# gpuopenanalytics/libgdf

Measured on AMD Instinct MI355X. Metric: hash-join probe rows/s, higher is better.
Workload: dtype int64

## Files before the change

### include/gdf/gdf_amd_testhook.h

```cpp
#ifndef GDF_AMD_TESTHOOK_H
#define GDF_AMD_TESTHOOK_H
#include "gdf/gdf.h"
#ifdef __cplusplus
extern "C" {
#endif
gdf_error gdf_amd_debug_force(const char *name, const char *value);
const char *gdf_amd_testhook_forced(const char *name);
void gdf_amd_testhook_note(const char *name, long long value);
gdf_error gdf_amd_debug_noted(const char *name, long long *value);
#ifdef __cplusplus
}
#endif
#endif
```

### libgdf_amd/csrc/join.hip

```cpp
#include "internal.h"
#include "launch.h"
#include "gdf/gdf_amd_ext.h"

#include <cmath>
#include <cstdio>

#include <algorithm>
#include <cstdlib>
#include <deque>
#include <memory>
#include <type_traits>
#include <vector>

namespace gdf_amd {

enum KeyMode : int { KM_RAW_INT = 0, KM_RAW_FLOAT, KM_PACKED, KM_HASHED };

struct KeyPlan {
  int mode;
  int verify;
  int narrow;
  uint64_t kmin;
  uint64_t kspan;
  uint64_t klimit;
  uint64_t kwindow;
  int shift[MAX_KEY_COLS];
  int ranged;
  int bits[MAX_KEY_COLS];
  long long bias[MAX_KEY_COLS];
};

static KeyPlan plan_keys(const KeyTable &t) {
  KeyPlan p{};
  bool all_int = true;
  int total = 0;
  for (int c = 0; c < t.ncols; ++c) {
    if (t.col[c].kind == K_F32 || t.col[c].kind == K_F64) all_int = false;
    p.shift[c] = total * 8;
    total += t.col[c].width;
  }
  if (t.ncols == 1) p.mode = all_int ? KM_RAW_INT : KM_RAW_FLOAT;
  else if (all_int && total <= 8) p.mode = KM_PACKED;
  else { p.mode = KM_HASHED; p.verify = 1; }
  if (p.mode != KM_HASHED && total <= 4) p.narrow = 1;
  p.klimit = p.narrow ? 0xffffffffULL : ~0ULL;
  return p;
}

__device__ __forceinline__ bool float_bits(const ColView &c, int64_t i, uint64_t &bits) {
  if (c.kind == K_F32) {
    uint32_t b = ((const uint32_t *)c.data)[i];
    if ((b & 0x7fffffffu) > 0x7f800000u) return false;
    if ((b << 1) == 0) b = 0;
    bits = b;
  } else {
    uint64_t b = ((const uint64_t *)c.data)[i];
    if ((b & 0x7fffffffffffffffULL) > 0x7ff0000000000000ULL) return false;
    if ((b << 1) == 0) b = 0;
    bits = b;
  }
  return true;
}

__device__ __forceinline__ long long load_int_signed(const ColView &c, int64_t i) {
  switch (c.width) {
    case 1: return ((const int8_t *)c.data)[i];
    case 2: return ((const int16_t *)c.data)[i];
    case 4: return ((const int32_t *)c.data)[i];
    default: return ((const long long *)c.data)[i];
  }
}

__device__ __forceinline__ bool make_key(const KeyTable &t, const KeyPlan &p, int64_t i, uint64_t &key) {
  if (!row_valid(t, i)) return false;
  switch (p.mode) {
    case KM_RAW_INT: {
      const uint64_t k = load_bits(t.col[0], i) - p.kmin;
      key = k;
      return k <= p.klimit;
    }
    case KM_RAW_FLOAT: return float_bits(t.col[0], i, key);
    case KM_PACKED: {
      uint64_t k = 0;
// ... 815 lines not shown
    uint32_t claimed = 0;
    {
      const uint32_t tid = opaque_tid();
      if (g.cap1 && tid < ncoarse) {
        const uint32_t cnt = s.hist[tid];
        if (cnt) claimed = atomicAdd(&g.spec_cursor1[(tid << g.xs) | (blockIdx.x & ((1u << g.xs) - 1u))], cnt);
      }
      tile_scan_bins(s, ncoarse, tid);
      block_sync();
    }
    const uint32_t wtid = opaque_tid();
    {
      uint32_t st[ITEMS];
#pragma unroll
      for (int k = 0; k < ITEMS; ++k) st[k] = s.start[(binrank[k] >> 16) & 255u];
#pragma unroll
      for (int k = 0; k < ITEMS; ++k) {
        const uint32_t pos = (okmask >> k) & 1u ? st[k] + (binrank[k] & 0xffffu) : (uint32_t)TILE;
        const int32_t row = g.row_base + (int32_t)(tile + item_row(k, wtid));
        s.w[pos] = ((uint64_t)key[k] << 32) | (uint32_t)row;
        if constexpr (PMODE == 4) *reinterpret_cast<ulonglong2 *>(&s.pay[2 * (size_t)pos]) = ulonglong2{pay[k], pay2[k]};
        else s.pay[pos] = pay[k];
      }
    }
    {
      const uint32_t tid = opaque_tid();
      if (tid < ncoarse) {
        if (g.cap1) {
          const uint32_t cnt = s.hist[tid];
          const uint32_t region = (tid << g.xs) | (blockIdx.x & ((1u << g.xs) - 1u));
          if (claimed + cnt > g.cap1) { atomicExch(g.spec_flag, 1u); s.gbase[tid] = g.dump - s.start[tid]; }
          else s.gbase[tid] = region * g.cap1 + claimed - s.start[tid];
        } else {
          s.gbase[tid] = s.cursor[tid] - s.start[tid];
          s.cursor[tid] += s.hist[tid];
        }
      }
      if (tid < 256) s.hist[tid] = 0;
      if (g.cap1 && tid == 0) s.total_abort = __hip_atomic_load(g.spec_flag, __ATOMIC_RELAXED, __HIP_MEMORY_SCOPE_AGENT);
    }
    const bool more = tile + TILE < end;
    __builtin_amdgcn_sched_barrier(0);
    if (more) prefetch(tile + TILE);
    block_sync();
    if (g.cap1 && s.total_abort) return;
    const uint32_t total = s.total;
    const uint32_t ftid = opaque_tid();
    constexpr int GROUP = ITEMS % 4 == 0 ? 4 : 3;
#pragma unroll
    for (int h = 0; h < ITEMS / GROUP; ++h) {
      uint64_t ww[GROUP], pp[GROUP], pq[PMODE == 4 ? GROUP : 1];
      uint32_t gb[GROUP];
#pragma unroll
      for (int k = 0; k < GROUP; ++k) {
        const uint32_t j = ftid + (h * GROUP + k) * THREADS;
        ww[k] = s.w[j];
        if constexpr (PMODE == 4) { const ulonglong2 e = *reinterpret_cast<const ulonglong2 *>(&s.pay[2 * (size_t)j]); pp[k] = e.x; pq[k] = e.y; }
        else pp[k] = s.pay[j];
      }
#pragma unroll
      for (int k = 0; k < GROUP; ++k) gb[k] = s.gbase[(fine_of((ww[k] >> 32) + g.kbias, g.fb) >> g.b2) & 255u];
#pragma unroll
      for (int k = 0; k < GROUP; ++k) {
        const uint32_t j = ftid + (h * GROUP + k) * THREADS;
        const uint32_t dst = j < total ? gb[k] + j : g.dump + ftid;
        out.w[dst] = ww[k];
        if constexpr (PMODE == 4) *reinterpret_cast<ulonglong2 *>(out.pay + 2 * (size_t)dst) = ulonglong2{pp[k], pq[k]};
        else out.pay[dst] = pp[k];
      }
      __builtin_amdgcn_sched_barrier(0);
    }
    consume(tile + TILE);
    __builtin_amdgcn_sched_barrier(0);
  }
}

struct Level2Map {
  const uint32_t *coarse_off;
  const uint32_t *coarse_end;
  const uint32_t *tile_prefix;
  int xs;
  uint32_t ntiles;
  int xcd_order;
  const uint32_t *ntiles_dev;
  uint32_t nseg;
  const uint32_t *keys32;
  uint32_t calib_step;
};
static inline uint32_t sc2_grid(const Level2Map &m, uint32_t ntiles) {
  const uint32_t tiles = m.calib_step > 1 ? (ntiles + m.calib_step - 1) / m.calib_step : ntiles;
  return m.xcd_order ? ((tiles + 7) / 8) * 8 : tiles;
}

template <bool NARROW, int THREADS, int PAY = 0, bool P6 = false, bool K32 = false, bool IN6 = false, int NITEMS = 0>
__global__ __launch_bounds__(THREADS) void jk_scatter2(PartGeom g, Level2Map m, Tuples in,
                                                             uint32_t *__restrict__ fine_cursor, Tuples out) {
  extern __shared__ __attribute__((aligned(16))) unsigned char tile_raw[];
  constexpr int ITEMS = NITEMS ? NITEMS : (PAY ? JK_PAY_ITEMS : JK_SC_ITEMS);
  using Tile = TileLds<NARROW, THREADS, PAY, ITEMS>;
  Tile &s = *reinterpret_cast<Tile *>(tile_raw);
  constexpr int JK_TILE = THREADS * ITEMS;
  const uint32_t ncoarse = 1u << g.b1, nsub = 1u << g.b2;
  const uint32_t per_xcd = gridDim.x >> 3;
  const uint32_t tile_id = (m.xcd_order ? (blockIdx.x & 7u) * per_xcd + (blockIdx.x >> 3) : blockIdx.x) * (m.calib_step > 1 ? m.calib_step : 1u);
  if (tile_id >= (m.ntiles_dev ? *m.ntiles_dev : m.ntiles)) return;
  uint32_t lo = 0, hi = m.nseg ? m.nseg : (ncoarse << m.xs);
  while (hi - lo > 1) {
    const uint32_t mid = (lo + hi) >> 1;
    if (m.tile_prefix[mid] <= tile_id) lo = mid; else hi = mid;
  }
  const uint32_t p = m.nseg ? (lo >> 3) / g.world : (lo >> m.xs);
  const uint32_t begin = m.coarse_off[lo] + (tile_id - m.tile_prefix[lo]) * JK_TILE;
  const uint32_t pend = m.coarse_end[lo];
  const uint32_t end = begin + JK_TILE < pend ? begin + JK_TILE : pend;
  const uint32_t submask = nsub - 1;

  if (threadIdx.x < 256) s.hist[threadIdx.x] = 0;
  block_sync();
  uint64_t w[ITEMS], pay[PAY ? ITEMS : 1], pay2[PAY == 2 ? ITEMS : 1];
  const bool quads = K32 && end - begin == (uint32_t)JK_TILE;
  int32_t idx[ITEMS];
  uint32_t live6 = 0;
  if constexpr (IN6) {
    static_assert(!IN6 || (P6 && !PAY && !K32), "six-byte input: the main path only");
    const uint32_t region = lo & ((1u << m.xs) - 1u);
    L6Pair d[ITEMS / 2];
    uint2 hw[NARROW ? 1 : ITEMS / 2];
#pragma unroll
    for (int k = 0; k < ITEMS / 2; ++k) {
      const uint32_t i = begin + 2u * (k * THREADS + threadIdx.x);
      const uint32_t ic = i < end ? i : end - 2u;
      d[k] = *reinterpret_cast<const L6Pair *>(reinterpret_cast<const unsigned char *>(in.w) + (size_t)ic * 6u);
      if constexpr (!NARROW) hw[k] = *reinterpret_cast<const uint2 *>(in.idx + ic);
    }
#pragma unroll
    for (int k = 0; k < ITEMS / 2; ++k) {
      uint32_t r0, w0, r1, w1;
      l6_unpack(d[k], r0, w0, r1, w1);
      const bool in_tile = begin + 2u * (k * THREADS + threadIdx.x) < end;
      const uint32_t all = (1u << (32 - g.b1)) - 1u;
      live6 |= (uint32_t)(in_tile && !(r0 == all && w0 == L6_ROW_MASK)) << (2 * k);
      live6 |= (uint32_t)(in_tile && !(r1 == all && w1 == L6_ROW_MASK)) << (2 * k + 1);
      w[2 * k] = ((uint64_t)((p << (32 - g.b1)) | r0) << 32) | (uint32_t)(g.row_base + (int32_t)l6_row(w0, region));
      w[2 * k + 1] = ((uint64_t)((p << (32 - g.b1)) | r1) << 32) | (uint32_t)(g.row_base + (int32_t)l6_row(w1, region));
      if constexpr (NARROW) idx[2 * k] = idx[2 * k + 1] = 0;
      else { idx[2 * k] = (int32_t)hw[k].x; idx[2 * k + 1] = (int32_t)hw[k].y; }
    }
  } else if (K32 && quads) {
    if constexpr (K32) {
#pragma unroll
      for (int q = 0; q < ITEMS / 4; ++q) {
        const uint32_t i0 = begin + 4u * (q * THREADS + threadIdx.x);
        const uint4 kk = *reinterpret_cast<const uint4 *>(m.keys32 + i0);
        w[4 * q + 0] = ((uint64_t)kk.x << 32) | (uint32_t)(g.row_base + (int32_t)i0);
        w[4 * q + 1] = ((uint64_t)kk.y << 32) | (uint32_t)(g.row_base + (int32_t)(i0 + 1));
        w[4 * q + 2] = ((uint64_t)kk.z << 32) | (uint32_t)(g.row_base + (int32_t)(i0 + 2));
        w[4 * q + 3] = ((uint64_t)kk.w << 32) | (uint32_t)(g.row_base + (int32_t)(i0 + 3));
        idx[4 * q] = idx[4 * q + 1] = idx[4 * q + 2] = idx[4 * q + 3] = 0;
      }
    }
  } else {
#pragma unroll
  for (int k = 0; k < ITEMS; ++k) {
    const uint32_t i = begin + k * THREADS + threadIdx.x;
    const uint32_t ic = i < end ? i : end - 1;
    if constexpr (K32) w[k] = ((uint64_t)m.keys32[ic] << 32) | (uint32_t)(g.row_base + (int32_t)ic);
    else w[k] = in.w[ic];
    idx[k] = NARROW ? 0 : in.idx[ic];
    if constexpr (PAY == 2) { const ulonglong2 e = *reinterpret_cast<const ulonglong2 *>(in.pay + 2 * (size_t)ic); pay[k] = e.x; pay2[k] = e.y; }
    else if (PAY) pay[k] = in.pay[ic];
  }
  }
  uint32_t binrank[ITEMS];
  const uint32_t kb_low = (uint32_t)g.kbias, kb_fold0 = (uint32_t)(g.kbias >> 32) * 0x9e3779b1u, kb_fold1 = kb_fold0 + 0x9e3779b1u;
  auto rank_tuples = [&](auto pow2_world) {
    constexpr bool POW2W = decltype(pow2_world)::value;
    const uint32_t wshift = POW2W ? (uint32_t)(31 - __clz((int)(g.world ? g.world : 1u))) : 0u;
#pragma unroll
    for (int k = 0; k < ITEMS; ++k) {
      const uint32_t i = begin + k * THREADS + threadIdx.x;
      if constexpr (IN6) {
        const uint32_t q = (uint32_t)(w[k] >> 32);
        binrank[k] = ((live6 >> k) & 1u) ? ((uint32_t)((uint64_t)q >> (32 - g.fb)) & submask) : 256u + (threadIdx.x & 63u);
        continue;
      }
      uint32_t q, lh;
      if constexpr (K32) {
        const uint32_t key32 = (uint32_t)(w[k] >> 32), low = key32 + kb_low;
        q = lowbias32(low ^ (low < key32 ? kb_fold1 : kb_fold0));
        lh = POW2W ? q << wshift : (uint32_t)((uint64_t)q * g.world);
      } else {
        q = hash_a(tup_key<NARROW>(w[k]) + g.kbias);
        lh = local_hash(q, g.world);
      }
      const uint32_t bin = (uint32_t)((uint64_t)lh >> (32 - g.fb)) & submask;
      binrank[k] = ((K32 && quads) || i < end) ? bin : 256u + (threadIdx.x & 63u);
      if constexpr (P6 && !NARROW) {
        const uint32_t row = (uint32_t)idx[k];
        idx[k] = (int32_t)(uint32_t)((w[k] + g.kbias) >> 32);
        w[k] = ((uint64_t)p6_low(q, lh, g.world) << 32) | row;
      } else if constexpr (P6) {
        if constexpr (K32 && POW2W) w[k] = ((uint64_t)(g.world > 1 ? __builtin_rotateleft32(q, wshift) : lh) << 32) | (uint32_t)w[k];
        else w[k] = ((uint64_t)p6_low(q, lh, g.world) << 32) | (uint32_t)w[k];
      }
    }
  };
  if (K32 && (g.world & (g.world - 1u)) == 0) rank_tuples(std::true_type{});
  else rank_tuples(std::false_type{});
#pragma unroll
  for (int k = 0; k < ITEMS; ++k)
    binrank[k] = (binrank[k] << 16) | atomicAdd(&s.hist[binrank[k]], 1u);
  block_sync();
  uint32_t claimed = 0, mine = 0;
  if (threadIdx.x < nsub) {
    mine = s.hist[threadIdx.x];
    if (mine) claimed = atomicAdd(&fine_cursor[(p << g.b2) | threadIdx.x], mine);
  }
  tile_scan_bins(s, nsub);
  block_sync();
#pragma unroll
  for (int h = 0; h < ITEMS; h += 8) {
    uint32_t st[8];
#pragma unroll
    for (int k = 0; k < 8; ++k) st[k] = s.start[(binrank[h + k] >> 16) & 255u];
#pragma unroll
    for (int k = 0; k < 8; ++k) {
      const uint32_t pos = (binrank[h + k] >> 24) ? (uint32_t)JK_TILE : st[k] + (binrank[h + k] & 0xffffu);
      s.w[pos] = w[h + k];
      if (!NARROW) s.idx[pos] = idx[h + k];
      if constexpr (PAY == 2) *reinterpret_cast<ulonglong2 *>(&s.pay[2 * (size_t)pos]) = ulonglong2{pay[h + k], pay2[h + k]};
      else if (PAY) s.pay[pos] = pay[h + k];
    }
  }
  if (threadIdx.x < nsub && mine) {
    const uint32_t f = (p << g.b2) | threadIdx.x;
    const uint32_t limit = g.fstart ? g.fstart[f] + g.fcap[f] : (f + 1) * g.cap2;
    if (g.cap2 && claimed + mine > limit) { atomicExch(g.spec_flag, 1u); s.gbase[threadIdx.x] = g.dump - s.start[threadIdx.x]; }
    else s.gbase[threadIdx.x] = claimed - s.start[threadIdx.x];
  }
  block_sync();
  tile_flush<false, NARROW, THREADS, PAY, ITEMS, P6>(s, g, out);
}

constexpr int JK_BK_THREADS = 1024;
template <class T>
__device__ __forceinline__ T bk_block_scan(T v, T *lds_wave, T *total) {
  const T incl = wave_scan_incl(v);
  block_sync();
  if (lane_id() == WAVE - 1) lds_wave[threadIdx.x / WAVE] = incl;
  block_sync();
  T woff = 0, tot = 0;
#pragma unroll
  for (int w = 0; w < JK_BK_THREADS / WAVE; ++w) {
    if (w < (int)(threadIdx.x / WAVE)) woff += lds_wave[w];
    tot += lds_wave[w];
  }
  *total = tot;
  return woff + incl - v;
}
constexpr uint32_t JK_L2MAP_LDS_SEGS = 16384;
__global__ __launch_bounds__(JK_BK_THREADS) void jk_make_l2map(const uint32_t *__restrict__ fill, uint32_t nseg, uint32_t cap1, uint32_t tile,
                                                               uint32_t *__restrict__ seg_begin, uint32_t *__restrict__ seg_end,
                                                               uint32_t *__restrict__ tile_prefix, uint32_t *__restrict__ ntiles,
                                                               uint32_t fj_world, uint32_t ncoarse, const uint32_t *__restrict__ rstart = nullptr,
                                                               const uint32_t *__restrict__ rcap = nullptr) {
  __shared__ uint32_t lds_wave[JK_BK_THREADS / WAVE];
  extern __shared__ __attribute__((aligned(16))) uint32_t l2map_lds[];
  const uint32_t per = (nseg + JK_BK_THREADS - 1) / JK_BK_THREADS;
  const uint32_t c0 = threadIdx.x * per;
  auto region_of = [&](uint32_t seg) -> uint32_t {
    if (!fj_world) return seg;
    const uint32_t cs = seg >> 3, c = cs / fj_world, sender = cs - c * fj_world;
    return ((sender * ncoarse + c) << 3) | (seg & 7u);
  };
  auto filled = [&](uint32_t region) -> uint32_t { const uint32_t n = fill[region], room = rcap ? rcap[region] : cap1; return n < room ? n : room; };
  const bool pow2 = (tile & (tile - 1u)) == 0;
  const int shift = __ffs((int)tile) - 1;
  auto tiles_of = [&](uint32_t n) -> uint32_t { return pow2 ? (n + tile - 1u) >> shift : (n + tile - 1u) / tile; };
  if (nseg <= JK_L2MAP_LDS_SEGS) {
    constexpr int MAXK = (int)(JK_L2MAP_LDS_SEGS / JK_BK_THREADS);
    uint32_t n_[MAXK], first_[MAXK];
#pragma unroll
    for (int k = 0; k < MAXK; ++k) {
      const uint32_t c = (uint32_t)k * JK_BK_THREADS + threadIdx.x;
      n_[k] = 0; first_[k] = 0;
      if (c < nseg) {
        const uint32_t r = region_of(c);
        n_[k] = filled(r);
        first_[k] = rstart ? rstart[r] : r * cap1;
        l2map_lds[c] = tiles_of(n_[k]);
      }
// ... 1449 lines not shown
  }
  ~SideBufs() { settle(); }
  Tuples tuples(int b) const { return Tuples{w[b].as<uint64_t>(), idx[b].as<int32_t>(), pay[b].as<uint64_t>()}; }
  Tuples final() const { return tuples(final_buf); }
};

static PartGeom choose_geometry(int64_t build_rows) {
  PartGeom g{};
  int fb = 0;
  while (fb < JK_MAX_FB && (build_rows >> fb) > JK_TARGET_BUILD) ++fb;
  if (fb < 5) fb = 5;
  if (const long long forced = lab::path_int("GDF_JK_FORCE_FB", 0)) { if (forced >= 5 && forced <= JK_MAX_FB) fb = (int)forced; }
  g.fb = fb;
  g.b1 = fb <= 8 ? fb : (fb + 1) / 2;
  g.b2 = fb - g.b1;
  g.b3 = 0;
  if (fb == JK_MAX_FB && !lab::path_on("GDF_JK_NO_LEVEL3"))
    while (g.b3 < 8 && (build_rows >> (fb + g.b3)) > JK_MAX_BUILD - JK_MAX_BUILD / 5) ++g.b3;
  return g;
}

static inline int small_grid(int64_t n) { return stream_grid((size_t)(n > 0 ? n : 1), 256 * 8); }

template <int FAST, bool NARROW, int THREADS, bool MASKED>
static gdf_error launch_scatter1_t(const KeyTable &t, const KeyPlan &plan, const PartGeom &g, const uint32_t *H1off, Tuples out) {
  const size_t lds = sizeof(TileLds<NARROW, THREADS, false, sc1_items(NARROW, THREADS)>);
  GDF_TRY(launch_lds("jk_scatter1", jk_scatter1<FAST, NARROW, THREADS, MASKED>, dim3(g.nchunks), dim3(THREADS), lds, t, plan, g, H1off, out));
  HIP_CHECK_LAST();
  return GDF_SUCCESS;
}
static constexpr int sc1_threads(bool narrow, int fast) { return (narrow || fast == 8) ? 1024 : 512; }
template <int FAST, bool NARROW, bool MASKED>
static gdf_error launch_scatter1_n(const KeyTable &t, const KeyPlan &plan, const PartGeom &g, const uint32_t *H1off, Tuples out) {
  return launch_scatter1_t<FAST, NARROW, sc1_threads(NARROW, FAST), MASKED>(t, plan, g, H1off, out);
}
static gdf_error launch_scatter1(int fast, bool narrow, const KeyTable &t, const KeyPlan &plan, const PartGeom &g,
                                 const uint32_t *H1off, Tuples out, bool l6 = false) {
  const bool masked = fast != 0 && t.col[0].valid != nullptr;
  if (l6) {
    if (!(fast && g.cap1 && g.xs == 6 && g.b1 == 8) || (!narrow && fast != 8)) return GDF_INVALID_API_CALL;
    if (!narrow) {
      const size_t lds = sizeof(TileLds<false, 1024, false, 12>);
      GDF_TRY(with_bools([&](auto M) {
        return launch_lds("jk_scatter1_w10", jk_scatter1<8, false, 1024, M(), true>, dim3(g.nchunks), dim3(1024), lds, t, plan, g, H1off, out);
      }, masked));
    } else {
      const size_t lds = sizeof(TileLds<true, 1024>);
      GDF_TRY(with_int<8, 4>(fast, [&](auto F) {
        return with_bools([&](auto M) {
          return launch_lds("jk_scatter1", jk_scatter1<F(), true, 1024, M(), true>, dim3(g.nchunks), dim3(1024), lds, t, plan, g, H1off, out);
        }, masked);
      }));
    }
    HIP_CHECK_LAST();
    return GDF_SUCCESS;
  }
  if (masked) {
    if (fast == 4) return launch_scatter1_n<4, true, true>(t, plan, g, H1off, out);
    return narrow ? launch_scatter1_n<8, true, true>(t, plan, g, H1off, out)
                  : launch_scatter1_n<8, false, true>(t, plan, g, H1off, out);
  }
  if (fast == 4) return launch_scatter1_n<4, true, false>(t, plan, g, H1off, out);
  if (fast == 8) return narrow ? launch_scatter1_n<8, true, false>(t, plan, g, H1off, out)
                               : launch_scatter1_n<8, false, false>(t, plan, g, H1off, out);
  return narrow ? launch_scatter1_n<0, true, false>(t, plan, g, H1off, out)
                : launch_scatter1_n<0, false, false>(t, plan, g, H1off, out);
}
static int fast_key_width(const KeyTable &t, const KeyPlan &plan) {
  if (t.ncols != 1 || (plan.mode != KM_RAW_INT && plan.mode != KM_RAW_FLOAT) || t.nrows < 2) return 0;
  if (t.col[0].valid && t.nrows < 64) return 0;
  if (t.col[0].width == 8) return 8;
  if (t.col[0].width == 4 && plan.narrow && plan.kmin == 0) return 4;
  return 0;
}
template <bool NARROW, int THREADS>
static constexpr size_t level2_lds_bytes() { using Tile = TileLds<NARROW, THREADS>; return offsetof(Tile, cursor); }
static gdf_error launch_scatter2(bool narrow, uint32_t ntiles, const PartGeom &g, Level2Map m, Tuples in,
                                 uint32_t *cursor, Tuples out, bool p6 = false, bool in6 = false, int pw = 1) {
  if (in6 && !(p6 && !m.keys32 && g.b1 == 8)) return GDF_INVALID_API_CALL;
  if (!in6 && p6 && !narrow && m.keys32) return GDF_INVALID_API_CALL;
  m.ntiles = ntiles;
  m.xcd_order = (ntiles >= 64 && !lab::path_on("GDF_JK_NO_XCD_ORDER")) ? 1 : 0;
  const uint32_t grid = sc2_grid(m, ntiles);
  auto launch = [&](const char *name, auto kernel, int threads, size_t lds) -> gdf_error {
    GDF_TRY(launch_lds(name, kernel, dim3(grid), dim3(threads), lds, g, m, in, cursor, out));
    HIP_CHECK_LAST();
    return GDF_SUCCESS;
  };
  if (in6) {
    if (!narrow)
      return launch("jk_scatter2_w10", jk_scatter2<false, 256, 0, true, false, true>, 256, level2_lds_bytes<false, 256>());
    return launch("jk_scatter2", jk_scatter2<true, 256, 0, true, false, true>, 256, sizeof(TileLds<true, 256>));
  }
  if (p6 && !narrow)
    return launch("jk_scatter2_w10", jk_scatter2<false, 256, 0, true>, 256, level2_lds_bytes<false, 256>());
  if (p6 || m.keys32) {
    const size_t lds = sizeof(TileLds<true, 256>);
    if (p6 && m.keys32) return launch("jk_scatter2", jk_scatter2<true, 256, 0, true, true>, 256, lds);
    if (p6) return launch("jk_scatter2", jk_scatter2<true, 256, 0, true, false>, 256, lds);
    return launch("jk_scatter2", jk_scatter2<true, 256, 0, false, true>, 256, lds);
  }
  if (narrow && in.pay && pw == 2) {
    using Tile = TileLds<true, 256, 2, JK_PAY_ITEMS>;
    return launch("jk_scatter2", jk_scatter2<true, 256, 2>, 256, offsetof(Tile, cursor));
  }
  if (narrow && in.pay)
    return launch("jk_scatter2", jk_scatter2<true, 256, 1>, 256, sizeof(TileLds<true, 256, true, JK_PAY_ITEMS>));
  if (narrow) return launch("jk_scatter2", jk_scatter2<true, JK_SC2_THREADS>, JK_SC2_THREADS, sizeof(TileLds<true, JK_SC2_THREADS>));
  return launch("jk_scatter2", jk_scatter2<false, JK_SC2_THREADS>, JK_SC2_THREADS, sizeof(TileLds<false, JK_SC2_THREADS>));
}

static gdf_error launch_scatter1_pay(int fast, int pmode, const KeyTable &t, const KeyPlan &plan, const PartGeom &g, const uint32_t *H1off,
                                     const PaySrc &ps, Tuples out) {
  GDF_TRY(with_int<8, 4>(fast, [&](auto F) {
    return with_int<1, 2, 3, 4>(pmode, [&](auto M) {
      const size_t lds = sizeof(TileLds<true, JK_PAY_THREADS, pay_words(M()), pay_items1(M())>);
      return launch_lds("jk_scatter1", jk_scatter1_pay<F(), M()>, dim3(g.nchunks), dim3(JK_PAY_THREADS), lds, t, plan, g, H1off, ps, out);
    });
  }));
  HIP_CHECK_LAST();
  return GDF_SUCCESS;
}

static gdf_error partition_side(const KeyTable &t, KeyPlan &plan, PartGeom g, SideBufs *sb, bool decide_narrow, const PaySrc *pay = nullptr,
                                int pmode = 0, bool device_index = false, bool want_p6 = false, bool keep_running = false) {
  const int64_t n = t.nrows;
  bool narrow = plan.narrow != 0;
  int64_t chunk = JK_CHUNK_ROWS;
  if (n / chunk > JK_MAX_CHUNKS) chunk = (n + JK_MAX_CHUNKS - 1) / JK_MAX_CHUNKS;
  constexpr int64_t MAX_TILE = 1024 * JK_SC_ITEMS;
  chunk = ((chunk + MAX_TILE - 1) / MAX_TILE) * MAX_TILE;
  g.chunk = chunk;
  g.nchunks = (int)((n + chunk - 1) / chunk);
  if (g.nchunks == 0) g.nchunks = 1;
  const uint32_t nfine = 1u << g.fb, ncoarse = 1u << g.b1;

  const int hist_grid = g.nchunks < NUM_CU ? g.nchunks : NUM_CU;
  const size_t hist_bytes = sizeof(uint32_t) * nfine + sizeof(long long) * 2 * (size_t)hist_grid;
  DevBuf fine_hist, H1;
  RMM_TRY(fine_hist.alloc(hist_bytes));
  RMM_TRY(H1.alloc(sizeof(uint32_t) * (size_t)ncoarse * g.nchunks));
  HIP_TRY(hipMemsetAsync(fine_hist.p, 0, sizeof(uint32_t) * nfine, stream0()));
  const size_t hist_lds = sizeof(uint32_t) * (nfine + ncoarse);
  const int fast = fast_key_width(t, plan);
  GDF_TRY(allow_lds(jk_hist<8>, hist_lds));
  GDF_TRY(allow_lds(jk_hist<4>, hist_lds));
  GDF_TRY(allow_lds(jk_hist<0>, hist_lds));
  long long *d_mm = nullptr;
  if (decide_narrow)
    d_mm = reinterpret_cast<long long *>(fine_hist.as<uint32_t>() + nfine);
  if (fast == 8)
    GDF_LAUNCH("jk_hist", jk_hist<8>, dim3(hist_grid), dim3(JK_HIST_THREADS), hist_lds, stream0(), t, plan, g,
               fine_hist.as<uint32_t>(), H1.as<uint32_t>(), d_mm);
  else if (fast == 4)
    GDF_LAUNCH("jk_hist", jk_hist<4>, dim3(hist_grid), dim3(JK_HIST_THREADS), hist_lds, stream0(), t, plan, g,
               fine_hist.as<uint32_t>(), H1.as<uint32_t>(), d_mm);
  else
    GDF_LAUNCH("jk_hist", jk_hist<0>, dim3(hist_grid), dim3(JK_HIST_THREADS), hist_lds, stream0(), t, plan, g,
               fine_hist.as<uint32_t>(), H1.as<uint32_t>(), d_mm);
  HIP_CHECK_LAST();
  std::vector<uint32_t> fh(hist_bytes / sizeof(uint32_t));
  ReadTicket hist_ticket;
  HIP_TRY(read_back_begin(&hist_ticket, fine_hist.p, d_mm ? hist_bytes : sizeof(uint32_t) * nfine, 0));
  DevBuf scan_a, scan_b, d_coarse, d_tiles, cursor;
  struct Quiesce { bool armed = true; ~Quiesce() { if (armed) (void)hipStreamSynchronize(stream0()); } } quiesce;
  GDF_TRY(scan_u32_async(H1.as<uint32_t>(), H1.as<uint32_t>(), (size_t)ncoarse * g.nchunks, false, &scan_a));
// ... 164 lines not shown
      const uint64_t cr = ((uint64_t)(Uc + 8.0 * std::sqrt(Uc) + 64.0) + 63) / 64 * 64;
      for (uint32_t r = 0; r < nreg; ++r) {
        rstart[c * nreg + r] = (uint32_t)std::min<uint64_t>(run1, 0xffffffffULL);
        rcap[c * nreg + r] = (uint32_t)std::min<uint64_t>(cr, 0x7fffffffULL);
        run1 += cr;
        max1 = std::max(max1, rcap[c * nreg + r]);
      }
    }
    size1 = run1 + JK_TILE;
    size2 = run2 + JK_TILE;
    cap1 = max1;
    cap2 = max2;
  }
  if (size1 >= 0x7fffffffULL || size2 >= 0x7fffffffULL) return GDF_SUCCESS;

  DevBuf spec;
  constexpr size_t ZERO_WORDS = 32;
  const size_t zero_at = ((size_t)nseg + 2) / 2 * 2;
  RMM_TRY(spec.alloc(sizeof(uint32_t) * (zero_at + ZERO_WORDS)));
  HIP_TRY(hipMemsetAsync(spec.p, 0, sizeof(uint32_t) * (zero_at + ZERO_WORDS), stream0()));
  g.kbias = plan.kmin;
  g.cap1 = cap1;
  g.cap2 = 0;
  g.dump = caps ? (uint32_t)(size1 - JK_TILE) : nseg * cap1;
  if (caps) {
    RMM_TRY(sb->d_caps.alloc(sizeof(uint32_t) * cap_words.size()));
    HIP_TRY(hipMemcpyAsync(sb->d_caps.p, cap_words.data(), sizeof(uint32_t) * cap_words.size(), hipMemcpyHostToDevice, stream0()));
    HIP_TRY(hipStreamSynchronize(stream0()));
    g.rstart = sb->d_caps.as<uint32_t>();
    g.rcap = g.rstart + nseg;
    g.fstart = g.rcap + nseg;
    g.fcap = g.fstart + nfine;
    sb->d_fstart = g.fstart;
    sb->d_fcap = g.fcap;
  }
  g.spec_cursor1 = spec.as<uint32_t>();
  g.spec_flag = spec.as<uint32_t>() + nseg;
  const bool placed = defer && !app && g.b2 > 0;
  const bool hi_placed1 = placed && l6 && !narrow;
  const size_t bytes1 = l6 ? 6 * ((size_t)size1 + 2048) + 16 : sizeof(uint64_t) * size1;
  const size_t bytes1_hi = sizeof(int32_t) * ((size_t)size1 + (l6 ? 2048 : 0));
  if (placed) RMM_TRY(sb->w[0].alloc_placed(JK_ROLE_LEVEL1, bytes1, place_draws_now(JK_PLACE_DRAWS)));
  else RMM_TRY(sb->w[0].alloc(bytes1));
  if (hi_placed1) RMM_TRY(sb->idx[0].alloc_placed(JK_ROLE_LEVEL1_HI, bytes1_hi, -1));
  else if (!narrow) RMM_TRY(sb->idx[0].alloc(bytes1_hi));
  const int pw = pay ? pay_words(pmode) : 1;
  sb->pay_words = pw;
  if (pay) RMM_TRY(sb->pay[0].alloc(sizeof(uint64_t) * pw * size1));
  if (placed) {
    for (int round = 0; round <= JK_PLACE_DRAWS && sb->w[0].measure; ++round) {
      PlaceRound charge;
      PartGeom gc = g;
      gc.nchunks = std::max(1, g.nchunks / 4);
      sb->w[0].clock_begin(stream0());
      if (pay) GDF_TRY(launch_scatter1_pay(fast, pmode, t, plan, gc, nullptr, *pay, sb->tuples(0)));
      else GDF_TRY(launch_scatter1(fast, narrow, t, plan, gc, nullptr, sb->tuples(0), l6));
      sb->w[0].clock_end(stream0());
      HIP_TRY(hipMemsetAsync(spec.p, 0, sizeof(uint32_t) * (nseg + 1), stream0()));
      RMM_TRY(sb->w[0].alloc_placed(JK_ROLE_LEVEL1, bytes1, place_draws_now(JK_PLACE_DRAWS)));
    }
    if (hi_placed1 && !sb->w[0].measure && place_budget_left()) RMM_TRY(sb->idx[0].alloc_placed(JK_ROLE_LEVEL1_HI, bytes1_hi, JK_PLACE_DRAWS));
    for (int round = 0; hi_placed1 && round <= JK_PLACE_DRAWS && sb->idx[0].measure; ++round) {
      PlaceRound charge;
      PartGeom gc = g;
      gc.nchunks = std::max(1, g.nchunks / 4);
      sb->idx[0].clock_begin(stream0());
      GDF_TRY(launch_scatter1(fast, narrow, t, plan, gc, nullptr, sb->tuples(0), l6));
      sb->idx[0].clock_end(stream0());
      HIP_TRY(hipMemsetAsync(spec.p, 0, sizeof(uint32_t) * (nseg + 1), stream0()));
      RMM_TRY(sb->idx[0].alloc_placed(JK_ROLE_LEVEL1_HI, bytes1_hi, place_draws_now(JK_PLACE_DRAWS)));
    }
  }
  DevBuf d_map, cursor;
  if (defer && !app && g.b2 > 0) {
    RMM_TRY(cursor.alloc(sizeof(uint32_t) * ((size_t)nfine + 2)));
    hipLaunchKernelGGL(jk_init_cursor, dim3(32), dim3(256), 0, stream0(), cursor.as<uint32_t>(), nfine, cap2, g.fstart);
    HIP_CHECK_LAST();
  }
  sb->w[0].clock_begin(stream0());
  if (pay) GDF_TRY(launch_scatter1_pay(fast, pmode, t, plan, g, nullptr, *pay, sb->tuples(0)));
  else GDF_TRY(launch_scatter1(fast, narrow, t, plan, g, nullptr, sb->tuples(0), l6));
  sb->w[0].clock_end(stream0());
  if (defer && !app && g.b2 > 0) {
    RMM_TRY(d_map.alloc(sizeof(uint32_t) * (3 * (size_t)nseg + 2)));
    uint32_t *seg_begin = d_map.as<uint32_t>(), *seg_end = seg_begin + nseg, *tile_prefix = seg_end + nseg;
    uint32_t *ntiles_dev = cursor.as<uint32_t>() + nfine + 1;
    size_t map_lds = 0;
    GDF_TRY(l2map_prepare(nseg, &map_lds));
    hipLaunchKernelGGL(jk_make_l2map, dim3(1), dim3(JK_BK_THREADS), map_lds, stream0(), (const uint32_t *)spec.as<uint32_t>(), nseg, cap1,
                       (uint32_t)JK_TILE2, seg_begin, seg_end, tile_prefix, ntiles_dev, 0u, 0u, g.rstart, g.rcap);
    HIP_CHECK_LAST();
    const bool p6 = want_p6 && !pay;
    const bool hi_inside2 = placed && p6 && !narrow;
    const size_t six2 = (6 * (size_t)size2 + 16 + 255) & ~(size_t)255;
    const size_t bytes2 = p6 ? (hi_inside2 ? six2 + sizeof(int32_t) * ((size_t)size2 + 2) : 6 * (size_t)size2 + 16) : sizeof(uint64_t) * size2;
    if (placed) RMM_TRY(sb->w[1].alloc_placed(JK_ROLE_LEVEL2, bytes2, place_draws_now(JK_PLACE_DRAWS_L2)));
    else RMM_TRY(sb->w[1].alloc(bytes2));
    if (hi_inside2) sb->idx[1].borrow(sb->w[1].as<char>() + six2);
    else if (!narrow) RMM_TRY(sb->idx[1].alloc(sizeof(int32_t) * size2));
    if (pay) RMM_TRY(sb->pay[1].alloc(sizeof(uint64_t) * pw * size2));
    PartGeom g2 = g;
    g2.cap2 = cap2;
    g2.dump = caps ? (uint32_t)(size2 - JK_TILE) : nfine * cap2;
    g2.spec_flag = cursor.as<uint32_t>() + nfine;
    Level2Map m{seg_begin, seg_end, tile_prefix, g.xs};
    m.ntiles_dev = ntiles_dev;
    const uint32_t tile_bound = (uint32_t)((uint64_t)n / (uint64_t)JK_TILE2) + nseg + 1;
    if (placed) {
      for (int round = 0; round <= JK_PLACE_DRAWS_L2 && sb->w[1].measure; ++round) {
        PlaceRound charge;
        Level2Map mc = m;
        mc.calib_step = 4;
        sb->w[1].clock_begin(stream0());
        GDF_TRY(launch_scatter2(narrow, tile_bound, g2, mc, sb->tuples(0), cursor.as<uint32_t>(), sb->tuples(1), p6, l6, pw));
        sb->w[1].clock_end(stream0());
        hipLaunchKernelGGL(jk_init_cursor, dim3(32), dim3(256), 0, stream0(), cursor.as<uint32_t>(), nfine, cap2, g.fstart);
        HIP_CHECK_LAST();
        RMM_TRY(sb->w[1].alloc_placed(JK_ROLE_LEVEL2, bytes2, place_draws_now(JK_PLACE_DRAWS_L2)));
        if (hi_inside2) sb->idx[1].borrow(sb->w[1].as<char>() + six2);
      }
    }
    sb->w[1].clock_begin(stream0());
    GDF_TRY(launch_scatter2(narrow, tile_bound, g2, m, sb->tuples(0), cursor.as<uint32_t>(), sb->tuples(1), p6, l6, pw));
    sb->w[1].clock_end(stream0());
    sb->p6 = p6;
    sb->d_map.p = d_map.release();
    sb->final_buf = 1;
    sb->fine_off.clear(); sb->fine_begin.clear(); sb->fine_cnt.clear();
    sb->deferred = true;
    sb->speculative = true;
    sb->cap2 = cap2;
    sb->nseg = nseg;
    sb->zero = reinterpret_cast<unsigned long long *>(spec.as<uint32_t>() + zero_at);
    sb->d_level1.p = spec.release();
    sb->d_cursor.p = cursor.release();
    *ok = true;
    return GDF_SUCCESS;
  }
  std::vector<uint32_t> c1(nseg + 1);
  HIP_TRY(read_back(c1.data(), spec.p, sizeof(uint32_t) * (nseg + 1)));
  if (c1[nseg]) return GDF_SUCCESS;
  sb->final_buf = 0;
  sb->fine_off.clear();
  if (app && g.b2 == 0) return GDF_SUCCESS;
  if (g.b2 == 0) {
    sb->fine_begin.resize(nfine);
    for (uint32_t f = 0; f < nfine; ++f) sb->fine_begin[f] = f * cap1;
    sb->fine_cnt.assign(c1.begin(), c1.begin() + nfine);
  } else {
    std::vector<uint32_t> coarse_off(2 * nseg), tile_prefix(nseg + 1), cur(nfine);
    tile_prefix[0] = 0;
    for (uint32_t c = 0; c < nseg; ++c) {
      coarse_off[c] = c * cap1;
      coarse_off[nseg + c] = c * cap1 + c1[c];
      tile_prefix[c + 1] = tile_prefix[c] + (uint32_t)((c1[c] + JK_TILE2 - 1) / JK_TILE2);
    }
    for (uint32_t f = 0; f < nfine; ++f) cur[f] = f * cap2;
    const uint32_t ntiles = tile_prefix[nseg];
    DevBuf d_coarse, d_tiles, own_cursor;
    DevBuf &cursor = app ? app->cursor : own_cursor;
    RMM_TRY(d_coarse.alloc(sizeof(uint32_t) * 2 * nseg));
    RMM_TRY(d_tiles.alloc(sizeof(uint32_t) * (nseg + 1)));
    HIP_TRY(hipMemcpyAsync(d_coarse.p, coarse_off.data(), sizeof(uint32_t) * 2 * nseg, hipMemcpyHostToDevice, stream0()));
    HIP_TRY(hipMemcpyAsync(d_tiles.p, tile_prefix.data(), sizeof(uint32_t) * (nseg + 1), hipMemcpyHostToDevice, stream0()));
    if (!app || !app->started) {
      RMM_TRY(cursor.alloc(sizeof(uint32_t) * ((size_t)nfine + 1)));
      cur.push_back(0u);
      HIP_TRY(hipMemcpyAsync(cursor.p, cur.data(), sizeof(uint32_t) * ((size_t)nfine + 1), hipMemcpyHostToDevice, stream0()));
      cur.pop_back();
      RMM_TRY(sb->w[1].alloc(sizeof(uint64_t) * size2));
      if (!narrow) RMM_TRY(sb->idx[1].alloc(sizeof(int32_t) * size2));
      if (pay) RMM_TRY(sb->pay[1].alloc(sizeof(uint64_t) * pw * size2));
      if (app) app->started = true;
    }
    PartGeom g2 = g;
    g2.cap2 = cap2;
    g2.dump = nfine * cap2;
    g2.spec_flag = cursor.as<uint32_t>() + nfine;
    Level2Map m{d_coarse.as<uint32_t>(), d_coarse.as<uint32_t>() + nseg, d_tiles.as<uint32_t>(), g.xs};
    if (ntiles) GDF_TRY(launch_scatter2(narrow, ntiles, g2, m, sb->tuples(0), cursor.as<uint32_t>(), sb->tuples(1), false, false, pw));
    uint32_t flag = 0;
    if (!app) {
      cur.resize((size_t)nfine + 1);
      HIP_TRY(read_back(cur.data(), cursor.p, sizeof(uint32_t) * ((size_t)nfine + 1)));
      flag = cur[nfine];
      cur.pop_back();
    } else {
      HIP_TRY(read_back(&flag, cursor.as<uint32_t>() + nfine, sizeof(uint32_t)));
    }
    sb->w[0].reset();
// ... 2048 lines not shown
```

### libgdf_amd/csrc/testhook.cpp

```cpp
#include <map>
#include <mutex>
#include <set>
#include <string>

#include "gdf/gdf_amd_testhook.h"

namespace {
std::mutex g_mutex;
std::map<std::string, const char *> &forced_map() { static std::map<std::string, const char *> m; return m; }
const char *intern(const char *value) { static std::set<std::string> pool; return pool.insert(value).first->c_str(); }
int g_count = 0;
std::map<std::string, long long> &note_map() { static std::map<std::string, long long> m; return m; }
}

extern "C" {

__attribute__((visibility("default"))) const char *gdf_amd_testhook_forced(const char *name) {
  if (__atomic_load_n(&g_count, __ATOMIC_RELAXED) == 0) return nullptr;
  std::lock_guard<std::mutex> lock(g_mutex);
  auto it = forced_map().find(name);
  return it == forced_map().end() ? nullptr : it->second;
}

__attribute__((visibility("default"))) gdf_error gdf_amd_debug_force(const char *name, const char *value) {
  if (!name) return GDF_INVALID_API_CALL;
  try {
    std::lock_guard<std::mutex> lock(g_mutex);
    auto &m = forced_map();
    if (value) m[name] = intern(value); else m.erase(name);
    __atomic_store_n(&g_count, (int)m.size(), __ATOMIC_RELAXED);
  } catch (...) {
    return GDF_MEMORYMANAGER_ERROR;
  }
  return GDF_SUCCESS;
}

__attribute__((visibility("default"))) void gdf_amd_testhook_note(const char *name, long long value) {
  if (!name) return;
  try {
    std::lock_guard<std::mutex> lock(g_mutex);
    note_map()[name] = value;
  } catch (...) {
  }
}

__attribute__((visibility("default"))) gdf_error gdf_amd_debug_noted(const char *name, long long *value) {
  std::lock_guard<std::mutex> lock(g_mutex);
  if (!value) { note_map().clear(); return GDF_SUCCESS; }
  if (!name) return GDF_INVALID_API_CALL;
  try {
    auto it = note_map().find(name);
    if (it == note_map().end()) return GDF_INVALID_API_CALL;
    *value = it->second;
  } catch (...) {
    return GDF_MEMORYMANAGER_ERROR;
  }
  return GDF_SUCCESS;
}

}
```

Baseline: 111.3 billion.

## Compute level-2 scatter tiles in closed form instead of building a segment map

```diff
diff --git a/include/gdf/gdf_amd_testhook.h b/include/gdf/gdf_amd_testhook.h
--- a/include/gdf/gdf_amd_testhook.h
+++ b/include/gdf/gdf_amd_testhook.h
@@ -8,6 +8,8 @@
 const char *gdf_amd_testhook_forced(const char *name);
 void gdf_amd_testhook_note(const char *name, long long value);
 gdf_error gdf_amd_debug_noted(const char *name, long long *value);
+int gdf_amd_debug_l2_tile(unsigned block, int xcd_order, unsigned calib_step, unsigned tile, unsigned nseg, const unsigned *fill,
+                          unsigned cap1, const unsigned *rstart, const unsigned *rcap, unsigned *grid, unsigned out[3]);
 #ifdef __cplusplus
 }
 #endif
diff --git a/libgdf_amd/csrc/join.hip b/libgdf_amd/csrc/join.hip
--- a/libgdf_amd/csrc/join.hip
+++ b/libgdf_amd/csrc/join.hip
@@ -1,4 +1,5 @@
 #include "internal.h"
+#include "l2tile.h"
 #include "launch.h"
 #include "gdf/gdf_amd_ext.h"
 
@@ -980,15 +981,14 @@
   int xs;
   uint32_t ntiles;
   int xcd_order;
+  uint32_t grid;
   const uint32_t *ntiles_dev;
   uint32_t nseg;
   const uint32_t *keys32;
   uint32_t calib_step;
+  uint32_t tiles_per_seg;
 };
-static inline uint32_t sc2_grid(const Level2Map &m, uint32_t ntiles) {
-  const uint32_t tiles = m.calib_step > 1 ? (ntiles + m.calib_step - 1) / m.calib_step : ntiles;
-  return m.xcd_order ? ((tiles + 7) / 8) * 8 : tiles;
-}
+static inline uint32_t sc2_grid(const Level2Map &m, uint32_t ntiles) { return l2_grid(ntiles, m.xcd_order, m.calib_step); }
 
 template <bool NARROW, int THREADS, int PAY = 0, bool P6 = false, bool K32 = false, bool IN6 = false, int NITEMS = 0>
 __global__ __launch_bounds__(THREADS) void jk_scatter2(PartGeom g, Level2Map m, Tuples in,
@@ -999,22 +999,26 @@
   Tile &s = *reinterpret_cast<Tile *>(tile_raw);
   constexpr int JK_TILE = THREADS * ITEMS;
   const uint32_t ncoarse = 1u << g.b1, nsub = 1u << g.b2;
-  const uint32_t per_xcd = gridDim.x >> 3;
-  const uint32_t tile_id = (m.xcd_order ? (blockIdx.x & 7u) * per_xcd + (blockIdx.x >> 3) : blockIdx.x) * (m.calib_step > 1 ? m.calib_step : 1u);
-  if (tile_id >= (m.ntiles_dev ? *m.ntiles_dev : m.ntiles)) return;
-  uint32_t lo = 0, hi = m.nseg ? m.nseg : (ncoarse << m.xs);
-  while (hi - lo > 1) {
-    const uint32_t mid = (lo + hi) >> 1;
-    if (m.tile_prefix[mid] <= tile_id) lo = mid; else hi = mid;
+  const uint32_t tile_id = l2_tile_id(blockIdx.x, m.grid, m.xcd_order, m.calib_step);
+  uint32_t lo = 0, begin = 0, end = 0;
+  if (m.tiles_per_seg) {
+    if (!l2_closed_tile(tile_id, m.tiles_per_seg, (uint32_t)JK_TILE, ncoarse << m.xs, g.spec_cursor1, g.cap1, g.rstart, g.rcap, &lo, &begin, &end))
+      return;
+  } else {
+    const uint32_t ntiles = m.ntiles_dev ? *m.ntiles_dev : m.ntiles;
+    uint32_t hi = m.nseg ? m.nseg : (ncoarse << m.xs);
+    while (hi - lo > 1) {
+      const uint32_t mid = (lo + hi) >> 1;
+      if (m.tile_prefix[mid] <= tile_id) lo = mid; else hi = mid;
+    }
+    const uint32_t first = m.coarse_off[lo], before = m.tile_prefix[lo], pend = m.coarse_end[lo];
+    if (tile_id >= ntiles) return;
+    begin = first + (tile_id - before) * JK_TILE;
+    end = begin + JK_TILE < pend ? begin + JK_TILE : pend;
   }
   const uint32_t p = m.nseg ? (lo >> 3) / g.world : (lo >> m.xs);
-  const uint32_t begin = m.coarse_off[lo] + (tile_id - m.tile_prefix[lo]) * JK_TILE;
-  const uint32_t pend = m.coarse_end[lo];
-  const uint32_t end = begin + JK_TILE < pend ? begin + JK_TILE : pend;
   const uint32_t submask = nsub - 1;
 
-  if (threadIdx.x < 256) s.hist[threadIdx.x] = 0;
-  block_sync();
   uint64_t w[ITEMS], pay[PAY ? ITEMS : 1], pay2[PAY == 2 ? ITEMS : 1];
   const bool quads = K32 && end - begin == (uint32_t)JK_TILE;
   int32_t idx[ITEMS];
@@ -1069,6 +1073,7 @@
     else if (PAY) pay[k] = in.pay[ic];
   }
   }
+  if (threadIdx.x < 256) s.hist[threadIdx.x] = 0;
   uint32_t binrank[ITEMS];
   const uint32_t kb_low = (uint32_t)g.kbias, kb_fold0 = (uint32_t)(g.kbias >> 32) * 0x9e3779b1u, kb_fold1 = kb_fold0 + 0x9e3779b1u;
   auto rank_tuples = [&](auto pow2_world) {
@@ -1105,6 +1110,7 @@
   };
   if (K32 && (g.world & (g.world - 1u)) == 0) rank_tuples(std::true_type{});
   else rank_tuples(std::false_type{});
+  block_sync();
 #pragma unroll
   for (int k = 0; k < ITEMS; ++k)
     binrank[k] = (binrank[k] << 16) | atomicAdd(&s.hist[binrank[k]], 1u);
@@ -2720,6 +2726,7 @@
   m.ntiles = ntiles;
   m.xcd_order = (ntiles >= 64 && !lab::path_on("GDF_JK_NO_XCD_ORDER")) ? 1 : 0;
   const uint32_t grid = sc2_grid(m, ntiles);
+  m.grid = grid;
   auto launch = [&](const char *name, auto kernel, int threads, size_t lds) -> gdf_error {
     GDF_TRY(launch_lds(name, kernel, dim3(grid), dim3(threads), lds, g, m, in, cursor, out));
     HIP_CHECK_LAST();
@@ -3050,14 +3057,25 @@
   else GDF_TRY(launch_scatter1(fast, narrow, t, plan, g, nullptr, sb->tuples(0), l6));
   sb->w[0].clock_end(stream0());
   if (defer && !app && g.b2 > 0) {
-    RMM_TRY(d_map.alloc(sizeof(uint32_t) * (3 * (size_t)nseg + 2)));
-    uint32_t *seg_begin = d_map.as<uint32_t>(), *seg_end = seg_begin + nseg, *tile_prefix = seg_end + nseg;
-    uint32_t *ntiles_dev = cursor.as<uint32_t>() + nfine + 1;
-    size_t map_lds = 0;
-    GDF_TRY(l2map_prepare(nseg, &map_lds));
-    hipLaunchKernelGGL(jk_make_l2map, dim3(1), dim3(JK_BK_THREADS), map_lds, stream0(), (const uint32_t *)spec.as<uint32_t>(), nseg, cap1,
-                       (uint32_t)JK_TILE2, seg_begin, seg_end, tile_prefix, ntiles_dev, 0u, 0u, g.rstart, g.rcap);
-    HIP_CHECK_LAST();
+    const uint32_t tiles_per_seg = (!caps && !lab::path_on("GDF_JK_L2_SEARCHED")) ? l2_tiles_per_seg(cap1, (uint32_t)JK_TILE2) : 0u;
+    Level2Map m{nullptr, nullptr, nullptr, g.xs};
+    uint32_t tile_bound = (uint32_t)((uint64_t)n / (uint64_t)JK_TILE2) + nseg + 1;
+    if (tiles_per_seg) {
+      m.tiles_per_seg = tiles_per_seg;
+      tile_bound = nseg * tiles_per_seg;
+      lab::note("jk.l2_closed_form", tiles_per_seg);
+    } else {
+      RMM_TRY(d_map.alloc(sizeof(uint32_t) * (3 * (size_t)nseg + 2)));
+      uint32_t *seg_begin = d_map.as<uint32_t>(), *seg_end = seg_begin + nseg, *tile_prefix = seg_end + nseg;
+      uint32_t *ntiles_dev = cursor.as<uint32_t>() + nfine + 1;
+      size_t map_lds = 0;
+      GDF_TRY(l2map_prepare(nseg, &map_lds));
+      GDF_LAUNCH("jk_make_l2map", jk_make_l2map, dim3(1), dim3(JK_BK_THREADS), map_lds, stream0(), (const uint32_t *)spec.as<uint32_t>(), nseg, cap1,
+                 (uint32_t)JK_TILE2, seg_begin, seg_end, tile_prefix, ntiles_dev, 0u, 0u, g.rstart, g.rcap);
+      HIP_CHECK_LAST();
+      m = Level2Map{seg_begin, seg_end, tile_prefix, g.xs};
+      m.ntiles_dev = ntiles_dev;
+    }
     const bool p6 = want_p6 && !pay;
     const bool hi_inside2 = placed && p6 && !narrow;
     const size_t six2 = (6 * (size_t)size2 + 16 + 255) & ~(size_t)255;
@@ -3071,9 +3089,6 @@
     g2.cap2 = cap2;
     g2.dump = caps ? (uint32_t)(size2 - JK_TILE) : nfine * cap2;
     g2.spec_flag = cursor.as<uint32_t>() + nfine;
-    Level2Map m{seg_begin, seg_end, tile_prefix, g.xs};
-    m.ntiles_dev = ntiles_dev;
-    const uint32_t tile_bound = (uint32_t)((uint64_t)n / (uint64_t)JK_TILE2) + nseg + 1;
     if (placed) {
       for (int round = 0; round <= JK_PLACE_DRAWS_L2 && sb->w[1].measure; ++round) {
         PlaceRound charge;
diff --git a/libgdf_amd/csrc/l2tile.h b/libgdf_amd/csrc/l2tile.h
--- /dev/null
+++ b/libgdf_amd/csrc/l2tile.h
@@ -0,0 +1,40 @@
+#pragma once
+#include <cstdint>
+
+#if defined(__HIPCC__) || defined(__CUDACC__)
+#define GDF_L2_HD __host__ __device__ __forceinline__
+#else
+#define GDF_L2_HD inline
+#endif
+
+namespace gdf_amd {
+
+GDF_L2_HD uint32_t l2_tiles_per_seg(uint32_t room, uint32_t tile) { return (room + tile - 1u) / tile; }
+
+GDF_L2_HD uint32_t l2_grid(uint32_t ntiles, int xcd_order, uint32_t calib_step) {
+  const uint32_t tiles = calib_step > 1 ? (ntiles + calib_step - 1u) / calib_step : ntiles;
+  return xcd_order ? ((tiles + 7u) / 8u) * 8u : tiles;
+}
+
+GDF_L2_HD uint32_t l2_tile_id(uint32_t block, uint32_t grid, int xcd_order, uint32_t calib_step) {
+  const uint32_t per_xcd = grid >> 3;
+  return (xcd_order ? (block & 7u) * per_xcd + (block >> 3) : block) * (calib_step > 1 ? calib_step : 1u);
+}
+
+GDF_L2_HD bool l2_closed_tile(uint32_t tile_id, uint32_t tiles_per_seg, uint32_t tile, uint32_t nseg, const uint32_t *fill, uint32_t cap1,
+                              const uint32_t *rstart, const uint32_t *rcap, uint32_t *seg, uint32_t *begin, uint32_t *end) {
+  const uint32_t s = tile_id / tiles_per_seg;
+  if (s >= nseg) return false;
+  const uint32_t n = fill[s];
+  const uint32_t room = rcap ? rcap[s] : cap1;
+  const uint32_t first = rstart ? rstart[s] : s * cap1;
+  const uint32_t off = (tile_id - s * tiles_per_seg) * tile;
+  const uint32_t used = n < room ? n : room;
+  if (off >= used) return false;
+  *seg = s;
+  *begin = first + off;
+  *end = first + (off + tile < used ? off + tile : used);
+  return true;
+}
+
+}
diff --git a/libgdf_amd/csrc/testhook.cpp b/libgdf_amd/csrc/testhook.cpp
--- a/libgdf_amd/csrc/testhook.cpp
+++ b/libgdf_amd/csrc/testhook.cpp
@@ -4,6 +4,7 @@
 #include <string>
 
 #include "gdf/gdf_amd_testhook.h"
+#include "l2tile.h"
 
 namespace {
 std::mutex g_mutex;
@@ -58,4 +59,15 @@
   return GDF_SUCCESS;
 }
 
+__attribute__((visibility("default"))) int gdf_amd_debug_l2_tile(unsigned block, int xcd_order, unsigned calib_step, unsigned tile, unsigned nseg,
+                                                                 const unsigned *fill, unsigned cap1, const unsigned *rstart, const unsigned *rcap,
+                                                                 unsigned *grid, unsigned out[3]) {
+  using namespace gdf_amd;
+  if (!fill || !out || !tile || !cap1) return 0;
+  const uint32_t T = l2_tiles_per_seg(cap1, tile), g = l2_grid(nseg * T, xcd_order, calib_step);
+  if (grid) *grid = g;
+  if (block >= g) return 0;
+  return l2_closed_tile(l2_tile_id(block, g, xcd_order, calib_step), T, tile, nseg, fill, cap1, rstart, rcap, &out[0], &out[1], &out[2]) ? 1 : 0;
 }
+
+}
```

After: 110.2 billion. 1.0% lower.
